# dan11003/CFEAR_Radarodometry_code_public

Hardware: AMD Instinct MI355X
Metric: radar scans/s (filter+feat+4-keyframe reg), 400x3360 polar (higher is better)
Workload: dtype u8 (filter) / f32+f64 (features, registration)

## Files before the change

cfear_radarodometry_code_public_amd/csrc/odometry_step_dev.h:

```cpp
#pragma once
#include "registration_dev.h"
#include "features_compact_dev.h"

#include <type_traits>

using namespace cfear_dev;

namespace cfear_dev {
constexpr int MAX_SCANS = 64;

struct BlockScratch {
  uint64_t* keys; float* spts; int* order; int* vstart; int* vlist;
  int* vcur;
  int* rng;
  double* part;
  int* tmpi;
  float* samples;
  double* match;
  int* assoc;
  int cap_points, p2cap, pair_cap;
  const int* vrank; const int* vperm;
};

struct SeqState {
// ... 65 lines not shown
                                                                          SeqState* states, const BlockScratch* scratch, double* cov_work,
                                                                          cfear_reg_summary* summaries, double* poses_out, cfear_sweep_record* records, hipStream_t stream);
#define CFEAR_LAUNCH_REG_BY_COST(KERNEL, P, count, st, ...)                                                                                          \
  do {                                                                                                                                               \
    if ((P).phase_times) hipLaunchKernelGGL((KERNEL<true, -1>), dim3(count), dim3(BLOCK_R), 0, st, P, __VA_ARGS__);                                   \
    else if ((P).rp.cost == CFEAR_COST_P2L) hipLaunchKernelGGL((KERNEL<false, CFEAR_COST_P2L>), dim3(count), dim3(BLOCK_R), 0, st, P, __VA_ARGS__);  \
    else if ((P).rp.cost == CFEAR_COST_P2D) hipLaunchKernelGGL((KERNEL<false, CFEAR_COST_P2D>), dim3(count), dim3(BLOCK_R), 0, st, P, __VA_ARGS__);  \
    else hipLaunchKernelGGL((KERNEL<false, CFEAR_COST_P2P>), dim3(count), dim3(BLOCK_R), 0, st, P, __VA_ARGS__);                                     \
  } while (0)

namespace {

constexpr int BLOCK_F = CFEAR_FEAT_BLOCK;
constexpr int BLOCK_R = CFEAR_REG_BLOCK;
static_assert(BLOCK_R >= 64 * CFEAR_EVAL_WAVES, "the controller sums the partial results of CFEAR_EVAL_WAVES waves unconditionally");
static_assert(CFEAR_REG_MAX_SCANS <= MAX_SCANS, "a registration cannot have more scans than a sequence keeps");
static_assert(FeatLdsC::total <= 80384, "two feature workgroups per compute unit");
struct RegLds {
  static constexpr size_t red_d = 0;
  static constexpr size_t par = red_d + 10 * CFEAR_RED_STRIDE * sizeof(double);
  static constexpr size_t red_i = par + 3 * CFEAR_REG_MAX_SCANS * sizeof(double);
  static constexpr size_t scanptr = red_i + 64 * sizeof(int);
  static constexpr size_t regsh = scanptr + CFEAR_REG_MAX_SCANS * sizeof(void*);
  static constexpr size_t total = (regsh + sizeof(RegShared) + 15) / 16 * 16;
};

#ifndef CFEAR_REG_LDS_BUDGET
#define CFEAR_REG_LDS_BUDGET 53760
#endif
static_assert(RegLds::total + sizeof(double) * CFEAR_MATCH_LDS_DOUBLES <= CFEAR_REG_LDS_BUDGET,
              "registration kernels: more than 53,760 B of LDS costs the third workgroup per compute unit");

__device__ inline int next_pow2(int n) { int p = 1; while (p < n) p <<= 1; return p; }

__device__ __forceinline__ FeatureScratch make_fscratch(const BlockScratch& B, unsigned char* lds) {
  FeatureScratch W;
  W.keys = B.keys; W.spts = B.spts; W.order = B.order; W.vstart = B.vstart; W.vlist = B.vlist;
  W.vcur = B.vcur; W.lds = false; W.tab_voxels = 0;
  W.rng = B.rng; W.part = B.part; W.tmpi = B.tmpi;
  W.cap = B.cap_points;
  W.vrank = B.vrank; W.vperm = B.vperm;
  W.samples = B.samples;
  W.red_i = reinterpret_cast<int*>(lds + FeatLdsC::red_i);
  W.red_f = reinterpret_cast<float*>(lds + FeatLdsC::red_f);
  return W;
}
__device__ inline void kd_build_block(ScanDev* S, const BlockScratch& B) {
  __syncthreads();
  if (threadIdx.x == 0) {
    const int frames = (int)(((size_t)7 * B.cap_points * sizeof(double)) / sizeof(KdFrame));
    const bool ok = S->kd.nodes && kd_build_serial(&S->kd, S->mean_f, S->n_cells, reinterpret_cast<KdFrame*>(B.part), frames);
    if (!ok && S->status == 0) S->status = CFEAR_ERR_UNSUPPORTED;
  }
  __syncthreads();
}
__device__ __forceinline__ void features_dispatch(ScanDev* S, int n, const FeatureParams& P, const BlockScratch& B,
                                                  unsigned char* lds, PhaseTimer* pt, const float* bounds, bool zeroed, bool byte_intensities,
                                                  const PointRegs& PR, bool registers_only = false) {
  const FeatureScratch W = make_fscratch(B, lds);
  if (!(byte_intensities && !W.vrank && features_block_c(S, n, P, W, lds, pt, bounds, zeroed, PR))) {
    if (registers_only && PR.rounds > 0) point_regs_to_global(PR, S->xyi);
    features_block(S, n, P, W, next_pow2(n), pt, bounds);
  }
  if (P.nn_tie == 2) kd_build_block(S, B);
}
__device__ inline RegScratch make_rscratch(const BlockScratch& B, unsigned char* lds) {
// ... 116 lines not shown
      sum->success = 0; sum->usable = 0; sum->outer_iterations = 0; sum->num_residuals = 0; sum->num_residual_blocks = 0;
      double v[3]; aff_to_xyt(st->Tcurrent, v);
      poses_out[3 * q] = v[0]; poses_out[3 * q + 1] = v[1]; poses_out[3 * q + 2] = v[2];
      if (OP.records) {
        cfear_sweep_record* r = OP.records + q;
        r->pose[0] = v[0]; r->pose[1] = v[1]; r->pose[2] = v[2]; r->final_cost = 0;
        r->outer_iterations = 0; r->num_residuals = 0; r->n_keyframes = 1; r->n_cells = cur->n_cells;
        for (int i = 0; i < 8; i++) r->inner_iterations[i] = 0;
      }
    }
    return;
  }
  ScanDev** sp = reinterpret_cast<ScanDev**>(lds + RegLds::scanptr);
  double* poses = reinterpret_cast<double*>(lds + RegLds::par);
  const int ns = nkf + 1;
  if (tid < nkf) {
    sp[tid] = slot_ptr(my_ring);
    double v[3]; aff_to_xyt(my_kf_pose, v);
    poses[3 * tid] = v[0]; poses[3 * tid + 1] = v[1]; poses[3 * tid + 2] = v[2];
  }
  if (tid == 0) {
    sp[ns - 1] = cur;
    double v[3]; aff_to_xyt(Tguess, v);
    poses[3 * (ns - 1)] = v[0]; poses[3 * (ns - 1) + 1] = v[1]; poses[3 * (ns - 1) + 2] = v[2];
  }
  if (tid >= 64 && tid < 100) cov_work[(size_t)q * 36 + (tid - 64)] = ((tid - 64) % 7 == 0) ? 1.0 : 0.0;
  __syncthreads();
  const RegScratch RW = make_rscratch(B, lds);
  register_block<KCOST>(sp, ns, poses, cov_work + (size_t)q * 36, OP.rp, RW, reinterpret_cast<double*>(lds + RegLds::par),
                 reinterpret_cast<RegShared*>(lds + RegLds::regsh), sum, TIMED ? &pt : nullptr,
                 (fopt & SEQ_FUSER_SOFT) ? cov_work + (size_t)q * 36 : nullptr, seq_row(OP, q));
  __syncthreads();
  if (TIMED) pt.mark();
  if (tid == 0) {
    if (OP.cs.ctx) {
      CovSampleCtx* c = OP.cs.ctx + q;
      c->n = ns; c->itr = sum->outer_iterations; c->num_residuals = sum->num_residuals; c->final_cost = sum->final_cost;
      c->soft = reinterpret_cast<const RegShared*>(lds + RegLds::regsh)->prior_on;
      for (int i = 0; i < nkf; i++) c->slot[i] = st->ring[i];
      c->slot[ns - 1] = cur_slot;
      for (int i = 0; i < 3 * ns; i++) c->pose[i] = poses[i];
    }
    Aff2 Tcurrent = aff_from_xyt(poses[3 * (ns - 1)], poses[3 * (ns - 1) + 1], poses[3 * (ns - 1) + 2]);
    const Aff2 Tpi = aff_inv(T_prev);
    const Aff2 Tmot_current = aff_mul(Tpi, Tcurrent);
    {
      const double dt = 0.25, lim = 200;
      const double vel = sqrt(Tmot_current.t0 * Tmot_current.t0 + Tmot_current.t1 * Tmot_current.t1) / dt;
      const double ax = (Tmot_current.t0 - TprevMot.t0) / (dt * dt), ay = (Tmot_current.t1 - TprevMot.t1) / (dt * dt);
      const double acc = sqrt(ax * ax + ay * ay);
      if (acc > lim || vel > lim) Tcurrent = Tguess;
    }
    st->Tmot = aff_mul(Tpi, Tcurrent);
    st->Tcurrent = Tcurrent;
    const Aff2 Tkeydiff = aff_mul(aff_inv(st->kf_pose[nkf - 1]), Tcurrent);
    bool fuse = true;
    const SeqRow row = seq_row(OP, q);
    if (row ? row->use_keyframe : OP.use_keyframe) {
      const double tn = sqrt(Tkeydiff.t0 * Tkeydiff.t0 + Tkeydiff.t1 * Tkeydiff.t1);
      const double rot = fabs(atan2(Tkeydiff.l2, Tkeydiff.l3));
      const double kd = row ? row->min_keyframe_dist : OP.min_keyframe_dist, kr = row ? row->min_keyframe_rot_deg : OP.min_keyframe_rot_deg;
      fuse = (tn > kd) || (rot > kr * 3.14159265358979323846 / 180.0);
    }
    if (fuse) {
      int m = nkf;
      st->ring[m] = cur_slot; st->kf_pose[m] = Tcurrent; m++;
      int freed;
      if (m > (row ? (row->shape >> 2) : OP.submap)) {
        freed = st->ring[0];
        for (int i = 0; i + 1 < m; i++) { st->ring[i] = st->ring[i + 1]; st->kf_pose[i] = st->kf_pose[i + 1]; }
        m--;
      } else {
        freed = m;
      }
      st->nkf = m; st->free_slot = freed;
    }
    st->T_prev = Tcurrent;
    st->frames++; st->last_slot = cur_slot;
    double v[3]; aff_to_xyt(Tcurrent, v);
    poses_out[3 * q] = v[0]; poses_out[3 * q + 1] = v[1]; poses_out[3 * q + 2] = v[2];
    if (OP.records) {
      cfear_sweep_record* r = OP.records + q;
      r->pose[0] = v[0]; r->pose[1] = v[1]; r->pose[2] = v[2]; r->final_cost = sum->final_cost;
      r->outer_iterations = sum->outer_iterations; r->num_residuals = sum->num_residuals; r->n_keyframes = st->nkf; r->n_cells = cur->n_cells;
      for (int i = 0; i < 8; i++) r->inner_iterations[i] = sum->inner_iterations[i];
    }
    if (OP.work) {
      const RegShared* rs = reinterpret_cast<const RegShared*>(lds + RegLds::regsh);
      int evals = 0;
      for (int i = 0; i < rs->nrec; i++) evals += rs->orec[i].inner;
      const int nsrc = rs->kf[ns - 1].n_cells;
      OP.work[q] = (unsigned)evals * (unsigned)rs->M + 6u * (unsigned)rs->nrec * (unsigned)(nkf * nsrc);
    }
    if (!TIMED && OP.wg_times) OP.wg_times[(size_t)q * 32 + 15] = (long long)wall_clock64();
  }
}


#ifndef CFEAR_REG_MIN_WG
#define CFEAR_REG_MIN_WG 3
#endif
#ifdef CFEAR_REG_NUM_VGPR
#define CFEAR_REG_VGPR_ATTR __attribute__((amdgpu_num_vgpr(CFEAR_REG_NUM_VGPR)))
#else
#define CFEAR_REG_VGPR_ATTR
#endif
template <bool TIMED, int KCOST>
__global__ __launch_bounds__(BLOCK_R, CFEAR_REG_MIN_WG) CFEAR_REG_VGPR_ATTR void register_step_kernel(OdoParams OP, SeqState* states, ScanDev* const* ,
                                                                const BlockScratch* scratch, double* ,
                                                                double* cov_work , cfear_reg_summary* summaries,
                                                                double* poses_out ) {
  __shared__ __attribute__((aligned(16))) unsigned char lds[RegLds::total];
  register_step_body<TIMED, KCOST>(lds, OP.order ? OP.order[blockIdx.x] : OP.seq0 + (int)blockIdx.x, OP, states, scratch, cov_work, summaries, poses_out);
}

}
```

cfear_radarodometry_code_public_amd/csrc/register_step.hip:

```cpp
#define CFEAR_REG_MAX_SCANS 8
#ifndef CFEAR_MATCH_LDS_CAP
#define CFEAR_MATCH_LDS_CAP 784
#endif
#include "common.h"
#include "odometry_step_dev.h"

static_assert(CFEAR_REG_MAX_SCANS == CFEAR_STEP_SMALL_SCANS, "common.h tells pipeline.hip when to launch these kernels");

void cfear_launch_register_step_small(const OdoParams& P, int count, hipStream_t st, SeqState* states, const BlockScratch* scratch, double* cov_work,
                                      cfear_reg_summary* summaries, double* poses_out) {
  CFEAR_LAUNCH_REG_BY_COST(register_step_kernel, P, count, st, states, nullptr, scratch, nullptr, cov_work, summaries, poses_out);
}
```

cfear_radarodometry_code_public_amd/csrc/registration_dev.h:

```cpp
#pragma once
#include "features_dev.h"

namespace cfear_dev {

struct RegParams {
  int cost, loss, weight_opt;
  int recompute_repeats;
  double loss_limit, covar_scale, regularization, assoc_radius;
  int max_outer, min_itr, max_inner;
  int nn_tie;
};

struct SeqParams {
  double loss_limit, covar_scale, regularization, min_keyframe_dist, min_keyframe_rot_deg;
  float radius;
  int weight_intensity, loss, weight_opt, max_outer, min_itr, max_inner, compensate, use_keyframe;
  int z_min;
  int source;
  int fuser;
  int k;
  int shape;
};
static_assert(sizeof(SeqParams) <= 96, "a row of the per-sequence table: 96 bytes at the most");
constexpr int seq_shape_pack(int cost, int submap) { return (cost & 3) | (submap << 2); }
// ... 135 lines not shown
#ifndef CFEAR_EVAL_WAVES
#define CFEAR_EVAL_WAVES 4
#endif
#ifndef CFEAR_REG_BLOCK
#define CFEAR_REG_BLOCK 256
#endif

enum { REG_CMD_BUILD = 1, REG_CMD_EVAL = 2, REG_CMD_DONE = 3 };
enum { REG_ST_BUILD = 0, REG_ST_LM_IT0 = 1, REG_ST_LM_CAND = 2, REG_ST_COV = 3 };

struct RegIo {
  double* poses; double* cov6; cfear_reg_summary* out; double* par; int n;
};

struct RegShared {
  int cmd, itr, M, state;
  int lds_match, assoc_path;
  double x[3];
  double c, s;
  double cur_c, cur_s, prev_c, prev_s;
  double Ttar[CFEAR_REG_MAX_SCANS][6];
  double Trel[CFEAR_REG_MAX_SCANS][6];
  GridView kf[CFEAR_REG_MAX_SCANS];
  const double* srs; long long scc;
  RegParams rp; RegScratch rw; RegIo rio;
  int prior_on, pad_p; double pL[9], pguess[3], palpha;
  int success, nres, ret, pad0;
  double xcur[3], prev_par[3], tsrc_last[3], prev_score;
  SolveSummary ss;
  NormalEq E;
  NormalEq G;
  double x_cost, x_norm, sc0, sc1, sc2, radius, decrease_factor, dg0, dg1, dg2, xc[3], model_cost_change;
  int reuse_diagonal, num_invalid, iteration, nrec;
  int moved, pad_m;
  struct OuterRec { int inner, term; double cost, pose[3]; } orec[8];
};
#define CFEAR_OUTER_LDS 8

typedef __attribute__((address_space(3))) RegShared LRegShared;
typedef __attribute__((address_space(3))) NormalEq LNormalEq;
typedef __attribute__((address_space(3))) double lds_f64;
__device__ __forceinline__ NormalEq neq_load(const LNormalEq* p) {
  NormalEq e; e.cost = p->cost; e.g0 = p->g0; e.g1 = p->g1; e.g2 = p->g2; e.h00 = p->h00; e.h01 = p->h01; e.h02 = p->h02;
  e.h11 = p->h11; e.h12 = p->h12; e.h22 = p->h22;
  return e;
}
__device__ __forceinline__ void neq_store(LNormalEq* p, const NormalEq& e) {
  p->cost = e.cost; p->g0 = e.g0; p->g1 = e.g1; p->g2 = e.g2; p->h00 = e.h00; p->h01 = e.h01; p->h02 = e.h02;
  p->h11 = e.h11; p->h12 = e.h12; p->h22 = e.h22;
}
#define CFEAR_GENERIC(T, lvalue) (*(T*)&(lvalue))

#ifndef CFEAR_MATCH_LDS_CAP
#define CFEAR_MATCH_LDS_CAP 622
#endif
#define CFEAR_MATCH_LDS_DOUBLES (8 * CFEAR_MATCH_LDS_CAP)
struct MatchPtrs { double *tmx, *tmy, *a0, *a1, *a2, *sx, *sy, *w; };
__device__ __forceinline__ MatchPtrs match_ptrs(double* base, size_t cap) {
  MatchPtrs m;
  m.tmx = base; m.tmy = base + cap; m.a0 = base + 2 * cap; m.a1 = base + 3 * cap; m.a2 = base + 4 * cap;
  m.sx = base + 5 * cap; m.sy = base + 6 * cap; m.w = base + 7 * cap;
  return m;
}
__device__ __forceinline__ double* lds_match_base() {
  __shared__ double s_match[CFEAR_MATCH_LDS_DOUBLES];
  return s_match;
}
__device__ __forceinline__ constexpr int match_lds_arrays(int cost) { return cost == CFEAR_COST_P2D ? 8 : (cost == CFEAR_COST_P2L ? 7 : 5); }
__device__ __forceinline__ constexpr int match_lds_cap(int cost) {
  return cost == CFEAR_COST_P2D ? CFEAR_MATCH_LDS_DOUBLES / 8 : (cost == CFEAR_COST_P2L ? CFEAR_MATCH_LDS_DOUBLES / 7 : CFEAR_MATCH_LDS_DOUBLES / 5);
}
__device__ __forceinline__ constexpr int match_lds_idx(int cost, int q) {
  return cost == CFEAR_COST_P2D ? q
       : cost == CFEAR_COST_P2L ? (q < 4 ? q : (q == 4 ? -1 : q - 1))
                                : (q < 2 ? q : (q < 5 ? -1 : q - 3));
}
static_assert(match_lds_idx(CFEAR_COST_P2L, 2) == 2 && match_lds_idx(CFEAR_COST_P2L, 3) == 3 && match_lds_idx(CFEAR_COST_P2L, 4) == -1 &&
              match_lds_idx(CFEAR_COST_P2L, 5) == 4 && match_lds_idx(CFEAR_COST_P2L, 6) == 5 && match_lds_idx(CFEAR_COST_P2L, 7) == 6, "P2L layout");
static_assert(match_lds_idx(CFEAR_COST_P2P, 2) == -1 && match_lds_idx(CFEAR_COST_P2P, 4) == -1 && match_lds_idx(CFEAR_COST_P2P, 5) == 2 &&
              match_lds_idx(CFEAR_COST_P2P, 6) == 3 && match_lds_idx(CFEAR_COST_P2P, 7) == 4, "P2P layout");
static_assert(match_lds_idx(CFEAR_COST_P2D, 4) == 4 && match_lds_idx(CFEAR_COST_P2D, 7) == 7, "P2D layout");
__device__ __forceinline__ MatchPtrs match_ptrs_lds(int cost) {
  double* base = lds_match_base();
  const size_t cap = (size_t)match_lds_cap(cost);
  auto at = [&](int q) -> double* { const int i = match_lds_idx(cost, q); return i < 0 ? nullptr : base + (size_t)i * cap; };
  MatchPtrs m;
  m.tmx = at(0); m.tmy = at(1); m.a0 = at(2); m.a1 = at(3); m.a2 = at(4); m.sx = at(5); m.sy = at(6); m.w = at(7);
  return m;
}

enum { CFEAR_LOSSK_ANY = 0, CFEAR_LOSSK_HUBER = 1, CFEAR_LOSSK_CAUCHY = 2 };
template <int SRC, int COST, int LOSSK>
__device__ __forceinline__ void evaluate_partial_t(const LRegShared* ls, int M, double x0, double x1, double c, double s,
                                                   double* res_out, int res_cap) {
  const int wave = threadIdx.x >> 6;
  if (wave >= CFEAR_EVAL_WAVES) return;
  typedef __attribute__((address_space(3))) const double lds_cdouble;
  struct Rd {
    lds_cdouble* l; const double* g; size_t cap;
    __device__ __forceinline__ double operator()(int arr, int i) const {
      if (SRC == 1) return l[match_lds_idx(COST, arr) * match_lds_cap(COST) + i];
      if (SRC == 0) return g[arr * cap + i];
      return i < match_lds_cap(COST) ? l[match_lds_idx(COST, arr) * match_lds_cap(COST) + i] : g[arr * cap + i];
    }
  } rd;
  rd.l = (lds_cdouble*)lds_match_base(); rd.g = ls->rw.tmx; rd.cap = (size_t)ls->rw.cap;
  const double loss_limit = ls->rp.loss_limit;
  const double cauchy_b = loss_limit * loss_limit, cauchy_c = 1.0 / cauchy_b;
  const int nthr = min(CFEAR_REG_BLOCK, CFEAR_EVAL_WAVES * 64);
  NormalEq a = {0, 0, 0, 0, 0, 0, 0, 0, 0, 0};
  if (!res_out) {
    constexpr int nr = (COST == CFEAR_COST_P2L) ? 1 : 2;
    struct Head { double r[2], J[2][3], w2, cost; };
    struct Raw { double v[8]; };
    typedef __attribute__((address_space(1))) const double g_cdouble;
    auto load = [&](int i) -> Raw {
      Raw r;
      constexpr int lc = match_lds_cap(COST);
      auto from_lds = [&]() {
#pragma unroll
        for (int q = 0; q < 8; q++) r.v[q] = match_lds_idx(COST, q) >= 0 ? rd.l[(match_lds_idx(COST, q) >= 0 ? match_lds_idx(COST, q) : 0) * lc + i] : 0.0;
      };
// ... 372 lines not shown
template <bool TC = false>
__device__ __noinline__ void emit_match(ScanDev* const* scans, const ScanDev* src, const LRegShared* sh, int nsrc, int p, int ti, int o, bool use_lds) {
  const RegParams& P = CFEAR_GENERIC(const RegParams, sh->rp);
  const RegScratch& W = CFEAR_GENERIC(const RegScratch, sh->rw);
  const int i = p / nsrc, j = p - i * nsrc;
  RCell cs = rcell_src(src, j);
  if (TC && P.cost != CFEAR_COST_P2P) { const TcMean u = tc_uncorrected_mean(src->rsrc, (size_t)src->cap_cells, j); cs.mx = u.x; cs.my = u.y; }
  RCell ct;
  {
    const double2* r = reinterpret_cast<const double2*>(sh->kf[i].rtar + 8 * (size_t)ti);
    const double2 r0 = r[0], r1 = r[1], r2 = r[2];
    ct.mx = r0.x; ct.my = r0.y; ct.nx = r1.x; ct.ny = r1.y; ct.ns = r2.x; ct.scale = r2.y;
  }
  const double* ctf = (P.cost == CFEAR_COST_P2D) ? scans[i]->rcov + 3 * (size_t)ti : nullptr;
  const double* Trel = (const double*)sh->Trel[i];
  const double* Ttar = (const double*)sh->Ttar[i];
  if (use_lds) write_match(match_ptrs_lds(P.cost), o, P, Trel, Ttar, cs, ct, ctf);
  else write_match(match_ptrs(W.tmx, (size_t)W.cap), o, P, Trel, Ttar, cs, ct, ctf);
}

struct Assoc4 { int t0, t1, t2, t3; };
__device__ __forceinline__ int assoc_get(const Assoc4& a, int i) { return i == 0 ? a.t0 : (i == 1 ? a.t1 : (i == 2 ? a.t2 : a.t3)); }

__device__ __noinline__ unsigned long long associate_cell4(const LRegShared* sh, int k0, int nk, int j, double curr_radius) {
  typedef __attribute__((address_space(1))) const double g_cf64;
  typedef unsigned u32x2 __attribute__((ext_vector_type(2)));
  typedef __attribute__((address_space(1))) const u32x2 g_cu32x2;
  typedef float f32x4 __attribute__((ext_vector_type(4)));
  typedef __attribute__((address_space(1))) const f32x4 g_cf32x4;
  typedef double f64x2 __attribute__((ext_vector_type(2)));
  typedef __attribute__((address_space(1))) const f64x2 g_cf64x2;
  constexpr int NC = 4;
  const double angle_outlier = 0.86602540378443864676;
  const size_t cc = (size_t)sh->scc;
  g_cf64* rs = (g_cf64*)sh->srs + j;
  const double mx = rs[0], my = rs[cc], snx = rs[2 * cc], sny = rs[3 * cc];
  const double m = curr_radius * (1.0 + 1e-6) + 1e-6;
  float qx[4], qy[4];
  int nrows[4];
  unsigned wide = 0;
  u32x2 L[4], H[4];
#pragma unroll
  for (int u = 0; u < 4; u++) {
    const int i = k0 + min(u, nk - 1);
    const auto* T = sh->Trel[i];
    qx[u] = (float)((T[0] * mx + T[1] * my) + T[4]);
    qy[u] = (float)((T[2] * mx + T[3] * my) + T[5]);
    const int gw = sh->kf[i].gw, gh = sh->kf[i].gh, nc = sh->kf[i].n_cells;
    const double igc = sh->kf[i].igc, gmx = (double)sh->kf[i].gminx, gmy = (double)sh->kf[i].gminy;
    int ax0 = (int)floor(((double)qx[u] - m - gmx) * igc), ax1 = (int)floor(((double)qx[u] + m - gmx) * igc);
    int ay0 = (int)floor(((double)qy[u] - m - gmy) * igc), ay1 = (int)floor(((double)qy[u] + m - gmy) * igc);
    ax0 = max(ax0, 0); ay0 = max(ay0, 0); ax1 = min(ax1, gw - 1); ay1 = min(ay1, gh - 1);
    const bool ok = (u < nk) && nc > 0 && gw > 0 && ax0 <= ax1 && ay0 <= ay1;
    const bool wd = ok && (ay1 - ay0 > 2 || nc > CFEAR_GRID16_MAX);
    wide |= wd ? (1u << u) : 0u;
    const bool use = ok && !wd;
    nrows[u] = use ? ay1 - ay0 + 1 : 0;
    const int b0 = use ? ay0 * gw + ax0 : 0, b1 = use ? ay0 * gw + ax1 + 1 : 0;
    typedef __attribute__((address_space(1))) const unsigned short g_cu16;
    g_cu16* o16 = (g_cu16*)grid_off16(sh->kf[i].gs);
    const int gw2 = use ? gw : 0;
    L[u].x = (unsigned)o16[b0] | ((unsigned)o16[b0 + gw2] << 16); L[u].y = (unsigned)o16[b0 + 2 * gw2];
    H[u].x = (unsigned)o16[b1] | ((unsigned)o16[b1 + gw2] << 16); H[u].y = (unsigned)o16[b1 + 2 * gw2];
  }
  int ti[4];
  f64x2 tn[2];
  auto search = [&](int u0) {
    int lo[2][3], cnt[2][2], tot[2], kmax = 0;
#pragma unroll
// ... 65 lines not shown
    gate_load(2);
    gate(2);
  } else {
    gate(0);
    ti[2] = ti[3] = -1;
  }
  unsigned long long r = 0;
#pragma unroll
  for (int u = 0; u < 4; u++) r |= (unsigned long long)(unsigned)(ti[u] & 0xFFFF) << (16 * u);
  return r;
}
__device__ __forceinline__ Assoc4 associate_cell(const ScanDev* src, const LRegShared* sh, int k0, int nk, int j, double curr_radius) {
  Assoc4 a;
  {
    const unsigned long long p = associate_cell4(sh, k0, nk, j, curr_radius);
    auto un = [](unsigned v) -> int { return v >= 0xFFFEu ? (int)v - 0x10000 : (int)v; };
    a.t0 = un((unsigned)(p & 0xFFFF)); a.t1 = un((unsigned)((p >> 16) & 0xFFFF)); a.t2 = un((unsigned)((p >> 32) & 0xFFFF)); a.t3 = un((unsigned)(p >> 48));
  }
  if (a.t0 == -2 || a.t1 == -2 || a.t2 == -2 || a.t3 == -2) {
    const int nsrc = src->n_cells;
    if (a.t0 == -2) a.t0 = associate_pair(src, sh, nsrc, (k0 + 0) * nsrc + j, curr_radius);
    if (a.t1 == -2) a.t1 = associate_pair(src, sh, nsrc, (k0 + 1) * nsrc + j, curr_radius);
    if (a.t2 == -2) a.t2 = associate_pair(src, sh, nsrc, (k0 + 2) * nsrc + j, curr_radius);
    if (a.t3 == -2) a.t3 = associate_pair(src, sh, nsrc, (k0 + 3) * nsrc + j, curr_radius);
  }
  return a;
}

template <int KCOST = -1, bool TC = false>
__device__ __forceinline__ void emit_cell(ScanDev* const* scans, const ScanDev* src, const LRegShared* sh,
                                          int nsrc, int k0, int nk, int j, Assoc4 a, unsigned long long pos, int mode ) {
  const int cost = KCOST >= 0 ? KCOST : __builtin_amdgcn_readfirstlane(sh->rp.cost), weight_opt = __builtin_amdgcn_readfirstlane(sh->rp.weight_opt);
  mode = __builtin_amdgcn_readfirstlane(mode);
  typedef __attribute__((address_space(1))) const double g_cf64;
  typedef double f64x2 __attribute__((ext_vector_type(2)));
  typedef __attribute__((address_space(1))) const f64x2 g_cf64x2;
  RCell cs;
  {
    const size_t cc = (size_t)sh->scc;
    g_cf64* r = (g_cf64*)sh->srs + j;
    cs.mx = r[0]; cs.my = r[cc]; cs.nx = r[2 * cc]; cs.ny = r[3 * cc]; cs.ns = r[4 * cc]; cs.scale = r[5 * cc];
    if (TC && cost != CFEAR_COST_P2P) { cs.mx = r[6 * cc]; cs.my = r[7 * cc]; }
  }
  (void)src;
  typedef __attribute__((address_space(3))) double lds_double;
  f64x2 R0[2], R1[2], R2[2];
#pragma unroll
  for (int i = 0; i < 4; i++) {
    if ((i & 1) == 0) {
      __builtin_amdgcn_sched_barrier(0);
#pragma unroll
      for (int u = 0; u < 2; u++) {
        const int tu = assoc_get(a, i + u);
        g_cf64x2* r = (g_cf64x2*)(sh->kf[k0 + min(i + u, nk - 1)].rtar + 8 * (size_t)(tu >= 0 ? tu : 0));
        R0[u] = r[0]; R1[u] = r[1]; R2[u] = r[2];
      }
    }
    const int ti = assoc_get(a, i);
    const bool on = ti >= 0 && i < nk;
    const int tix = on ? ti : 0;
    const int ki = k0 + min(i, nk - 1);
    const int o = (int)((pos >> (16 * i)) & 0xFFFF);
    lds_double* lm = (lds_double*)lds_match_base() + o;
    double* gm = sh->rw.tmx + o;
    const size_t gcap = (size_t)sh->rw.cap;
    const f64x2 r0 = R0[i & 1], r1 = R1[i & 1], r2 = R2[i & 1];
    const auto* T = sh->Trel[ki];
    const auto* Tt = sh->Ttar[ki];
    const double tmx = (Tt[0] * r0.x + Tt[1] * r0.y) + Tt[4];
    const double tmy = (Tt[2] * r0.x + Tt[3] * r0.y) + Tt[5];
    const double nx = T[0] * cs.nx + T[1] * cs.ny;
// ... 63 lines not shown
  }
  if (a.t0 >= 0 || a.t1 >= 0 || a.t2 >= 0 || a.t3 >= 0) emit_cell<KCOST, TC>(scans, src, sh, nsrc, k0, nk, j, a, before + e, mode);
  return tb;
}

template <int KCOST = -1, bool TC = false>
__device__ __noinline__ void emit_item(ScanDev* const* scans, const ScanDev* src, const LRegShared* sh, int nsrc, int k0, int nk, int j, int4 v,
                                       unsigned long long pos, int mode) {
  const Assoc4 a = {v.x, v.y, v.z, v.w};
  emit_cell<KCOST, TC>(scans, src, sh, nsrc, k0, nk, j, a, pos, mode);
}

template <int KCOST = -1, bool TC = false>
__device__ __forceinline__ int build_problem_block(ScanDev* const* scans, int n, LRegShared* sh, int itr) {
  const ScanDev* src = scans[n - 1];
  const int nsrc = sh->kf[n - 1].n_cells;
  const int pairs = (n - 1) * nsrc;
  const int nt = CFEAR_REG_BLOCK, tid = threadIdx.x;
  int M;
  int mode;
  const int nk = n - 1;
  const int ngroups = (nk + 3) >> 2;
  const int lcap = match_lds_cap(KCOST >= 0 ? KCOST : sh->rp.cost);
  const bool can_park = 6 * (long long)ngroups * nsrc <= (long long)sh->rw.acap && (reinterpret_cast<uintptr_t>(sh->rw.assoc) & 15) == 0;
  bool done = false;
  int assoc_path = 3;
  const int tie_rule = sh->rp.nn_tie;
  if (tie_rule == 0 && nk <= 4 && nsrc <= nt) {
    const AssocBlock R = assoc_block(src, sh, 0, nk, nsrc, itr, 0, 0, false);
    const unsigned long long T = R.tb;
    const unsigned long long t0 = T & 0xFFFF, t1 = (T >> 16) & 0xFFFF, t2 = (T >> 32) & 0xFFFF, t3 = (T >> 48) & 0xFFFF;
    M = (int)(t0 + t1 + t2 + t3);
    mode = M <= lcap ? 1 : 2;
    (void)emit_block<KCOST, TC>(scans, src, sh, 0, nk, nsrc, 0, 0, false, R.a, R.e, (t0 << 16) | ((t0 + t1) << 32) | ((t0 + t1 + t2) << 48), mode);
    done = true; assoc_path = 1;
  } else if (tie_rule == 0 && can_park && (long long)nk * nsrc <= 65535 && nk <= 64) {
    const double curr_radius = (itr == 1) ? 2 * sh->rp.assoc_radius : sh->rp.assoc_radius;
    const int nitems = ngroups * nsrc;
    int4* park = reinterpret_cast<int4*>(sh->rw.assoc);
    unsigned long long* ppos = reinterpret_cast<unsigned long long*>(sh->rw.assoc + 4 * (size_t)nitems);
    unsigned long long* gt = reinterpret_cast<unsigned long long*>(sh->rw.red_i);
    for (int it = tid; it < nitems; it += nt) {
      const int g = it / nsrc, j = it - g * nsrc;
      const Assoc4 a = associate_cell(src, sh, 4 * g, min(4, nk - 4 * g), j, curr_radius);
      park[it] = make_int4(a.t0, a.t1, a.t2, a.t3);
    }
    __syncthreads();
    {
      const int lane = lane_id(), wv = tid >> 6, nwv = nt >> 6;
      for (int g = wv; g < ngroups; g += nwv) {
        unsigned long long run = 0;
        for (int j0 = 0; j0 < nsrc; j0 += 64) {
          const int j = j0 + lane;
          const bool in = j < nsrc;
          const int4 v = in ? park[(size_t)g * nsrc + j] : make_int4(-1, -1, -1, -1);
          const unsigned long long b0 = __ballot(v.x >= 0), b1 = __ballot(v.y >= 0), b2 = __ballot(v.z >= 0), b3 = __ballot(v.w >= 0);
          const unsigned long long below = (1ull << lane) - 1ull;
          const unsigned long long e = (unsigned long long)__popcll(b0 & below) | ((unsigned long long)__popcll(b1 & below) << 16) |
                                       ((unsigned long long)__popcll(b2 & below) << 32) | ((unsigned long long)__popcll(b3 & below) << 48);
          if (in) ppos[(size_t)g * nsrc + j] = run + e;
          run += (unsigned long long)__popcll(b0) | ((unsigned long long)__popcll(b1) << 16) | ((unsigned long long)__popcll(b2) << 32) |
                 ((unsigned long long)__popcll(b3) << 48);
        }
        if (lane == 0) gt[g] = run;
      }
    }
    __syncthreads();
// ... 6 lines not shown
        base += t0 + t1 + t2 + t3;
      }
      gt[0] = base;
    }
    __syncthreads();
    M = (int)gt[0];
    mode = M <= lcap ? 1 : 2;
    for (int it = tid; it < nitems; it += nt) {
      const int g = it / nsrc, j = it - g * nsrc;
      const int4 v = park[it];
      if (v.x >= 0 || v.y >= 0 || v.z >= 0 || v.w >= 0) emit_item<KCOST, TC>(scans, src, sh, nsrc, 4 * g, min(4, nk - 4 * g), j, v, gt[16 + g] + ppos[it], mode);
    }
    done = true; assoc_path = 2;
  }
  if (!done) {
    const double curr_radius = (itr == 1) ? 2 * sh->rp.assoc_radius : sh->rp.assoc_radius;
    const int ipt = (pairs + nt - 1) / nt;
    const int p0 = tid * ipt, p1 = min(pairs, p0 + ipt);
    int cnt = 0;
    for (int p = p0; p < p1; p++) {
      const bool rule_ok = tie_rule == 0 || (size_t)sh->rw.cap * 64 >= (size_t)nt * CFEAR_KD_STACK * sizeof(KdVisit);
      if (!rule_ok) assoc_path = -3;
      const int ti = (tie_rule != 0 && rule_ok) ? associate_pair_rule(scans, src, sh, nsrc, p, curr_radius, tie_rule) : associate_pair(src, sh, nsrc, p, curr_radius);
      sh->rw.assoc[p] = ti;
      cnt += (ti >= 0) ? 1 : 0;
    }
    int o = block_exclusive_scan<CFEAR_REG_BLOCK>(cnt, sh->rw.red_i, &M);
    mode = M <= lcap ? 1 : 2;
    for (int p = p0; p < p1; p++) {
      const int ti = sh->rw.assoc[p];
      if (ti >= 0) { emit_match<TC>(scans, src, sh, nsrc, p, ti, o, mode == 1 || o < lcap); o++; }
    }
  }
  if (tid == 0) { sh->lds_match = mode; sh->assoc_path = assoc_path; }
  __syncthreads();
  return M;
}


__device__ __forceinline__ void ctl_publish_eval(LRegShared* sh, double x0, double x1, double x2, int state, double cs, double sn) {
  sh->x[0] = x0; sh->x[1] = x1; sh->x[2] = x2;
  sh->c = cs; sh->s = sn;
  sh->cmd = REG_CMD_EVAL; sh->state = state;
}
__device__ __forceinline__ void ctl_publish_eval_cur(LRegShared* sh, int state) {
  ctl_publish_eval(sh, sh->xcur[0], sh->xcur[1], sh->xcur[2], state, sh->cur_c, sh->cur_s);
}

__device__ __noinline__ void ctl_publish_candidate(LRegShared* sh) {
  const double x2 = sh->xc[2];
  double sn, cs;
  sincos(x2, &sn, &cs);
  ctl_publish_eval(sh, sh->xc[0], sh->xc[1], x2, REG_ST_LM_CAND, cs, sn);
}

__device__ __noinline__ void ctl_publish_build(LRegShared* sh, bool first) {
  const auto& io = sh->rio;
  const int n = io.n, L = 3 * (n - 1);
  Aff2 Tsrc;
  if (first) {
    Tsrc = aff_from_xyt(sh->xcur[0], sh->xcur[1], sh->xcur[2]);
    sh->cur_c = Tsrc.l0; sh->cur_s = Tsrc.l2; sh->prev_c = Tsrc.l0; sh->prev_s = Tsrc.l2;
  } else {
    const double cs = sh->cur_c, sn = sh->cur_s;
    Tsrc.l0 = cs; Tsrc.l1 = -sn; Tsrc.l2 = sn; Tsrc.l3 = cs; Tsrc.t0 = sh->xcur[0]; Tsrc.t1 = sh->xcur[1];
  }
  for (int i = lane_id(); i < n - 1; i += 64) {
// ... 291 lines not shown

template <int KCOST = -1, bool TC = false>
__device__ inline int register_block(ScanDev* const* scans, int n, double* poses, double* cov6, const RegParams& P_in,
                                     const RegScratch& W_in, double* par_lds, RegShared* sh, cfear_reg_summary* out,
                                     PhaseTimer* pt = nullptr, const double* prior_cov6 = nullptr, SeqRow row = nullptr) {
  const int tid = threadIdx.x;
  LRegShared* ls = (LRegShared*)sh;
  if (tid == 0) {
    sh->rp = P_in; sh->rw = W_in;
    seq_reg_params(sh->rp, row);
    sh->rio.poses = poses; sh->rio.cov6 = cov6; sh->rio.out = out; sh->rio.par = par_lds; sh->rio.n = n;
  }
  __syncthreads();
  const RegParams& P = CFEAR_GENERIC(const RegParams, sh->rp);
  const RegScratch& W = CFEAR_GENERIC(const RegScratch, sh->rw);
  const RegIo& io = sh->rio;
  const bool master = (tid >> 6) == 0;
  double last_in0 = 0, last_in1 = 0, last_in2 = 0;
  if (master) { last_in0 = poses[3 * (n - 1)]; last_in1 = poses[3 * (n - 1) + 1]; last_in2 = poses[3 * (n - 1) + 2]; }
  for (int i = tid; i < n; i += CFEAR_REG_BLOCK) {
    const Aff2 T = aff_from_xyt(poses[3 * i], poses[3 * i + 1], poses[3 * i + 2]);
    double v[3]; aff_to_xyt(T, v);
    par_lds[3 * i] = v[0]; par_lds[3 * i + 1] = v[1]; par_lds[3 * i + 2] = v[2];
  }
  for (int i = tid; i < n; i += CFEAR_REG_BLOCK) sh->kf[i] = grid_view(scans[i]);
  if (tid == 64) { sh->srs = scans[n - 1]->rsrc; sh->scc = (long long)scans[n - 1]->cap_cells; }
  if (tid == 0 && out) {
    out->success = 0; out->usable = 0; out->outer_iterations = 0; out->num_residuals = 0; out->num_residual_blocks = 0;
    out->assoc_path = 0; out->final_cost = 0; out->score = 0;
  }
  if (out)
    for (int i = tid; i < CFEAR_MAX_OUTER; i += CFEAR_REG_BLOCK) { out->inner_iterations[i] = 0; out->termination[i] = 0; out->outer_cost[i] = 0; out->outer_pose[i][0] = out->outer_pose[i][1] = out->outer_pose[i][2] = 0; }
  __syncthreads();
  if (master) {
    const int L = 3 * (n - 1);
    sh->xcur[0] = par_lds[L]; sh->xcur[1] = par_lds[L + 1]; sh->xcur[2] = par_lds[L + 2];
    sh->prior_on = 0;
    if (prior_cov6) {
      double pL[9];
      prior_sqrt_info(prior_cov6, pL);
      for (int k = 0; k < 9; k++) sh->pL[k] = pL[k];
      sh->pguess[0] = par_lds[L]; sh->pguess[1] = par_lds[L + 1]; sh->pguess[2] = par_lds[L + 2];
      sh->palpha = sqrt((double)scans[n - 1]->n_cells);
      sh->prior_on = 1;
    }
    sh->prev_par[0] = sh->xcur[0]; sh->prev_par[1] = sh->xcur[1]; sh->prev_par[2] = sh->xcur[2];
    sh->tsrc_last[0] = last_in0; sh->tsrc_last[1] = last_in1; sh->tsrc_last[2] = last_in2;
    sh->prev_score = 1.7976931348623157e308;
    sh->success = 1; sh->nres = 0; sh->M = 0; sh->ret = 0; sh->itr = 1; sh->nrec = 0;
    sh->moved = 1;
    sh->ss.num_iterations = 0; sh->ss.termination = 0; sh->ss.final_cost = 0; sh->ss.last_relative_decrease = 0;
    ctl_publish_build(ls, true);
  }
  long long* const acc2g = (pt && pt->acc2 && tid == 0) ? pt->acc2 : nullptr;
  long long ac[8] = {0, 0, 0, 0, 0, 0, 0, 0};
  long long* const acc2 = acc2g ? ac : nullptr;
  for (;;) {
    long long t0c = 0;
    if (pt && (pt->acc || acc2) && tid == 0) t0c = (long long)wall_clock64();
    __syncthreads();
    const int cmd = ls->cmd;
    if (cmd == REG_CMD_DONE) break;
    long long tb = 0;
    if (acc2) tb = (long long)wall_clock64();
    if (cmd == REG_CMD_BUILD) {
      if (pt) pt->mark();
// ... 72 lines not shown
```

Measured before the change: 2.002 million.

## Stage source cells in LDS tail and parallelize keyframe ring update

Measured after the change: 2.010 million, median of 6. About the same (+0.4%).

```diff
diff --git a/cfear_radarodometry_code_public_amd/csrc/odometry_step_dev.h b/cfear_radarodometry_code_public_amd/csrc/odometry_step_dev.h
--- a/cfear_radarodometry_code_public_amd/csrc/odometry_step_dev.h
+++ b/cfear_radarodometry_code_public_amd/csrc/odometry_step_dev.h
@@ -121,6 +121,18 @@
               "registration kernels: more than 53,760 B of LDS costs the third workgroup per compute unit");
 
 __device__ inline int next_pow2(int n) { int p = 1; while (p < n) p <<= 1; return p; }
+
+__device__ __forceinline__ double lane_f64(double v, int lane) {
+  const unsigned long long b = (unsigned long long)__double_as_longlong(v);
+  const unsigned lo = (unsigned)__builtin_amdgcn_readlane((int)(unsigned)b, lane), hi = (unsigned)__builtin_amdgcn_readlane((int)(unsigned)(b >> 32), lane);
+  return __longlong_as_double((long long)(((unsigned long long)hi << 32) | lo));
+}
+__device__ __forceinline__ Aff2 lane_aff(const Aff2& T, int lane) {
+  Aff2 R;
+  R.l0 = lane_f64(T.l0, lane); R.l1 = lane_f64(T.l1, lane); R.l2 = lane_f64(T.l2, lane); R.l3 = lane_f64(T.l3, lane);
+  R.t0 = lane_f64(T.t0, lane); R.t1 = lane_f64(T.t1, lane);
+  return R;
+}
 
 __device__ __forceinline__ FeatureScratch make_fscratch(const BlockScratch& B, unsigned char* lds) {
   FeatureScratch W;
@@ -303,6 +315,9 @@
                  (fopt & SEQ_FUSER_SOFT) ? cov_work + (size_t)q * 36 : nullptr, seq_row(OP, q));
   __syncthreads();
   if (TIMED) pt.mark();
+  if (tid >= 64) return;
+  const int ring_i = st->ring[tid];
+  const Aff2 kf_i = st->kf_pose[tid];
   if (tid == 0) {
     if (OP.cs.ctx) {
       CovSampleCtx* c = OP.cs.ctx + q;
@@ -312,40 +327,46 @@
       c->slot[ns - 1] = cur_slot;
       for (int i = 0; i < 3 * ns; i++) c->pose[i] = poses[i];
     }
-    Aff2 Tcurrent = aff_from_xyt(poses[3 * (ns - 1)], poses[3 * (ns - 1) + 1], poses[3 * (ns - 1) + 2]);
-    const Aff2 Tpi = aff_inv(T_prev);
-    const Aff2 Tmot_current = aff_mul(Tpi, Tcurrent);
-    {
-      const double dt = 0.25, lim = 200;
-      const double vel = sqrt(Tmot_current.t0 * Tmot_current.t0 + Tmot_current.t1 * Tmot_current.t1) / dt;
-      const double ax = (Tmot_current.t0 - TprevMot.t0) / (dt * dt), ay = (Tmot_current.t1 - TprevMot.t1) / (dt * dt);
-      const double acc = sqrt(ax * ax + ay * ay);
-      if (acc > lim || vel > lim) Tcurrent = Tguess;
-    }
+  }
+  Aff2 Tcurrent = aff_from_xyt(poses[3 * (ns - 1)], poses[3 * (ns - 1) + 1], poses[3 * (ns - 1) + 2]);
+  const Aff2 Tpi = aff_inv(T_prev);
+  const Aff2 Tmot_current = aff_mul(Tpi, Tcurrent);
+  {
+    const double dt = 0.25, lim = 200;
+    const double vel = sqrt(Tmot_current.t0 * Tmot_current.t0 + Tmot_current.t1 * Tmot_current.t1) / dt;
+    const double ax = (Tmot_current.t0 - TprevMot.t0) / (dt * dt), ay = (Tmot_current.t1 - TprevMot.t1) / (dt * dt);
+    const double acc = sqrt(ax * ax + ay * ay);
+    if (acc > lim || vel > lim) Tcurrent = Tguess;
+  }
+  if (tid == 0) {
     st->Tmot = aff_mul(Tpi, Tcurrent);
     st->Tcurrent = Tcurrent;
-    const Aff2 Tkeydiff = aff_mul(aff_inv(st->kf_pose[nkf - 1]), Tcurrent);
-    bool fuse = true;
-    const SeqRow row = seq_row(OP, q);
-    if (row ? row->use_keyframe : OP.use_keyframe) {
-      const double tn = sqrt(Tkeydiff.t0 * Tkeydiff.t0 + Tkeydiff.t1 * Tkeydiff.t1);
-      const double rot = fabs(atan2(Tkeydiff.l2, Tkeydiff.l3));
-      const double kd = row ? row->min_keyframe_dist : OP.min_keyframe_dist, kr = row ? row->min_keyframe_rot_deg : OP.min_keyframe_rot_deg;
-      fuse = (tn > kd) || (rot > kr * 3.14159265358979323846 / 180.0);
+  }
+  const Aff2 kf_last = lane_aff(kf_i, nkf - 1);
+  const Aff2 Tkeydiff = aff_mul(aff_inv(kf_last), Tcurrent);
+  bool fuse = true;
+  const SeqRow row = seq_row(OP, q);
+  if (row ? row->use_keyframe : OP.use_keyframe) {
+    const double tn = sqrt(Tkeydiff.t0 * Tkeydiff.t0 + Tkeydiff.t1 * Tkeydiff.t1);
+    const double rot = fabs(atan2(Tkeydiff.l2, Tkeydiff.l3));
+    const double kd = row ? row->min_keyframe_dist : OP.min_keyframe_dist, kr = row ? row->min_keyframe_rot_deg : OP.min_keyframe_rot_deg;
+    fuse = (tn > kd) || (rot > kr * 3.14159265358979323846 / 180.0);
+  }
+  int nkf_new = nkf;
+  if (fuse) {
+    if (tid == 0) { st->ring[nkf] = cur_slot; st->kf_pose[nkf] = Tcurrent; }
+    int freed;
+    if (nkf + 1 > (row ? (row->shape >> 2) : OP.submap)) {
+      freed = __builtin_amdgcn_readfirstlane(ring_i);
+      if (tid >= 1 && tid < nkf) { st->ring[tid - 1] = ring_i; st->kf_pose[tid - 1] = kf_i; }
+      if (tid == 0) { st->ring[nkf - 1] = cur_slot; st->kf_pose[nkf - 1] = Tcurrent; }
+    } else {
+      nkf_new = nkf + 1;
+      freed = nkf_new;
     }
-    if (fuse) {
-      int m = nkf;
-      st->ring[m] = cur_slot; st->kf_pose[m] = Tcurrent; m++;
-      int freed;
-      if (m > (row ? (row->shape >> 2) : OP.submap)) {
-        freed = st->ring[0];
-        for (int i = 0; i + 1 < m; i++) { st->ring[i] = st->ring[i + 1]; st->kf_pose[i] = st->kf_pose[i + 1]; }
-        m--;
-      } else {
-        freed = m;
-      }
-      st->nkf = m; st->free_slot = freed;
-    }
+    if (tid == 0) { st->nkf = nkf_new; st->free_slot = freed; }
+  }
+  if (tid == 0) {
     st->T_prev = Tcurrent;
     st->frames++; st->last_slot = cur_slot;
     double v[3]; aff_to_xyt(Tcurrent, v);
@@ -353,7 +374,7 @@
     if (OP.records) {
       cfear_sweep_record* r = OP.records + q;
       r->pose[0] = v[0]; r->pose[1] = v[1]; r->pose[2] = v[2]; r->final_cost = sum->final_cost;
-      r->outer_iterations = sum->outer_iterations; r->num_residuals = sum->num_residuals; r->n_keyframes = st->nkf; r->n_cells = cur->n_cells;
+      r->outer_iterations = sum->outer_iterations; r->num_residuals = sum->num_residuals; r->n_keyframes = nkf_new; r->n_cells = cur->n_cells;
       for (int i = 0; i < 8; i++) r->inner_iterations[i] = sum->inner_iterations[i];
     }
     if (OP.work) {
@@ -365,6 +386,7 @@
     }
     if (!TIMED && OP.wg_times) OP.wg_times[(size_t)q * 32 + 15] = (long long)wall_clock64();
   }
+  if (TIMED) pt.mark();
 }
 
 
diff --git a/cfear_radarodometry_code_public_amd/csrc/register_step.hip b/cfear_radarodometry_code_public_amd/csrc/register_step.hip
--- a/cfear_radarodometry_code_public_amd/csrc/register_step.hip
+++ b/cfear_radarodometry_code_public_amd/csrc/register_step.hip
@@ -1,4 +1,7 @@
 #define CFEAR_REG_MAX_SCANS 8
+#ifndef CFEAR_SRC_STAGE
+#define CFEAR_SRC_STAGE 1
+#endif
 #ifndef CFEAR_MATCH_LDS_CAP
 #define CFEAR_MATCH_LDS_CAP 784
 #endif
diff --git a/cfear_radarodometry_code_public_amd/csrc/registration_dev.h b/cfear_radarodometry_code_public_amd/csrc/registration_dev.h
--- a/cfear_radarodometry_code_public_amd/csrc/registration_dev.h
+++ b/cfear_radarodometry_code_public_amd/csrc/registration_dev.h
@@ -191,7 +191,8 @@
   NormalEq G;
   double x_cost, x_norm, sc0, sc1, sc2, radius, decrease_factor, dg0, dg1, dg2, xc[3], model_cost_change;
   int reuse_diagonal, num_invalid, iteration, nrec;
-  int moved, pad_m;
+  int moved;
+  int src_lds;
   struct OuterRec { int inner, term; double cost, pose[3]; } orec[8];
 };
 #define CFEAR_OUTER_LDS 8
@@ -247,6 +248,11 @@
   m.tmx = at(0); m.tmy = at(1); m.a0 = at(2); m.a1 = at(3); m.a2 = at(4); m.sx = at(5); m.sy = at(6); m.w = at(7);
   return m;
 }
+
+#ifndef CFEAR_SRC_STAGE
+#define CFEAR_SRC_STAGE 0
+#endif
+static_assert(!CFEAR_SRC_STAGE || CFEAR_REG_BLOCK > 64, "the waves behind the controller wave stage the source cells");
 
 enum { CFEAR_LOSSK_ANY = 0, CFEAR_LOSSK_HUBER = 1, CFEAR_LOSSK_CAUCHY = 2 };
 template <int SRC, int COST, int LOSSK>
@@ -685,9 +691,17 @@
   typedef __attribute__((address_space(1))) const f64x2 g_cf64x2;
   constexpr int NC = 4;
   const double angle_outlier = 0.86602540378443864676;
-  const size_t cc = (size_t)sh->scc;
-  g_cf64* rs = (g_cf64*)sh->srs + j;
-  const double mx = rs[0], my = rs[cc], snx = rs[2 * cc], sny = rs[3 * cc];
+  double mx, my, snx, sny;
+  const int slc = CFEAR_SRC_STAGE ? __builtin_amdgcn_readfirstlane(sh->src_lds) : 0;
+  if (CFEAR_SRC_STAGE && slc) {
+    typedef __attribute__((address_space(3))) const double lds_cf64;
+    lds_cf64* ls = (lds_cf64*)lds_match_base() + (slc - 1 - j);
+    mx = ls[0]; my = ls[slc]; snx = ls[2 * slc]; sny = ls[3 * slc];
+  } else {
+    const size_t cc = (size_t)sh->scc;
+    g_cf64* rs = (g_cf64*)sh->srs + j;
+    mx = rs[0]; my = rs[cc]; snx = rs[2 * cc]; sny = rs[3 * cc];
+  }
   const double m = curr_radius * (1.0 + 1e-6) + 1e-6;
   float qx[4], qy[4];
   int nrows[4];
@@ -819,11 +833,18 @@
                                           int nsrc, int k0, int nk, int j, Assoc4 a, unsigned long long pos, int mode ) {
   const int cost = KCOST >= 0 ? KCOST : __builtin_amdgcn_readfirstlane(sh->rp.cost), weight_opt = __builtin_amdgcn_readfirstlane(sh->rp.weight_opt);
   mode = __builtin_amdgcn_readfirstlane(mode);
+  const bool staged = CFEAR_SRC_STAGE && !TC && (mode & 4);
+  mode &= 3;
   typedef __attribute__((address_space(1))) const double g_cf64;
   typedef double f64x2 __attribute__((ext_vector_type(2)));
   typedef __attribute__((address_space(1))) const f64x2 g_cf64x2;
   RCell cs;
-  {
+  if (staged) {
+    typedef __attribute__((address_space(3))) const double lds_cf64;
+    const int slc = match_lds_cap(cost);
+    lds_cf64* ls = (lds_cf64*)lds_match_base() + (slc - 1 - j);
+    cs.mx = ls[0]; cs.my = ls[slc]; cs.nx = ls[2 * slc]; cs.ny = ls[3 * slc]; cs.ns = ls[4 * slc]; cs.scale = ls[5 * slc];
+  } else {
     const size_t cc = (size_t)sh->scc;
     g_cf64* r = (g_cf64*)sh->srs + j;
     cs.mx = r[0]; cs.my = r[cc]; cs.nx = r[2 * cc]; cs.ny = r[3 * cc]; cs.ns = r[4 * cc]; cs.scale = r[5 * cc];
@@ -953,7 +974,8 @@
     const unsigned long long t0 = T & 0xFFFF, t1 = (T >> 16) & 0xFFFF, t2 = (T >> 32) & 0xFFFF, t3 = (T >> 48) & 0xFFFF;
     M = (int)(t0 + t1 + t2 + t3);
     mode = M <= lcap ? 1 : 2;
-    (void)emit_block<KCOST, TC>(scans, src, sh, 0, nk, nsrc, 0, 0, false, R.a, R.e, (t0 << 16) | ((t0 + t1) << 32) | ((t0 + t1 + t2) << 48), mode);
+    const int staged = (CFEAR_SRC_STAGE && !TC && sh->src_lds != 0 && M + nsrc <= lcap) ? 4 : 0;
+    (void)emit_block<KCOST, TC>(scans, src, sh, 0, nk, nsrc, 0, 0, false, R.a, R.e, (t0 << 16) | ((t0 + t1) << 32) | ((t0 + t1 + t2) << 48), mode | staged);
     done = true; assoc_path = 1;
   } else if (tie_rule == 0 && can_park && (long long)nk * nsrc <= 65535 && nk <= 64) {
     const double curr_radius = (itr == 1) ? 2 * sh->rp.assoc_radius : sh->rp.assoc_radius;
@@ -1026,7 +1048,10 @@
       if (ti >= 0) { emit_match<TC>(scans, src, sh, nsrc, p, ti, o, mode == 1 || o < lcap); o++; }
     }
   }
-  if (tid == 0) { sh->lds_match = mode; sh->assoc_path = assoc_path; }
+  if (tid == 0) {
+    sh->lds_match = mode; sh->assoc_path = assoc_path;
+    if (CFEAR_SRC_STAGE && !TC && M + sh->kf[n - 1].n_cells > lcap) sh->src_lds = 0;
+  }
   __syncthreads();
   return M;
 }
@@ -1384,6 +1409,25 @@
   if (out)
     for (int i = tid; i < CFEAR_MAX_OUTER; i += CFEAR_REG_BLOCK) { out->inner_iterations[i] = 0; out->termination[i] = 0; out->outer_cost[i] = 0; out->outer_pose[i][0] = out->outer_pose[i][1] = out->outer_pose[i][2] = 0; }
   __syncthreads();
+  if (CFEAR_SRC_STAGE && !TC) {
+    const int cost = KCOST >= 0 ? KCOST : ls->rp.cost;
+    const int nsrc = ls->kf[n - 1].n_cells, lc = match_lds_cap(cost);
+    const bool stage = cost != CFEAR_COST_P2P && ls->rp.nn_tie == 0 && n - 1 <= 4 && nsrc > 0 && nsrc <= CFEAR_REG_BLOCK && nsrc <= lc;
+    if (stage && !master) {
+      typedef __attribute__((address_space(1))) const double g_cf64;
+      const size_t cc = (size_t)ls->scc;
+      for (int j = tid - 64; j < nsrc; j += CFEAR_REG_BLOCK - 64) {
+        g_cf64* r = (g_cf64*)ls->srs + j;
+        lds_f64* lm = (lds_f64*)lds_match_base() + (lc - 1 - j);
+        double v[6];
+#pragma unroll
+        for (int f = 0; f < 6; f++) v[f] = r[f * cc];
+#pragma unroll
+        for (int f = 0; f < 6; f++) lm[f * lc] = v[f];
+      }
+    }
+    if (tid == 0) ls->src_lds = stage ? lc : 0;
+  }
   if (master) {
     const int L = 3 * (n - 1);
     sh->xcur[0] = par_lds[L]; sh->xcur[1] = par_lds[L + 1]; sh->xcur[2] = par_lds[L + 2];
```
